# kije/gpu_raytracer

Measured on AMD Instinct MI355X. Metric: Mrays/s, higher is better.
Workload: dtype f32

## Files before the change

gpu_raytracer_amd/csrc/rt_frame.cpp:

```cpp
#include "rt_internal.h"

#ifndef RT_SINGLE_PASS_MAX_NODES
#define RT_SINGLE_PASS_MAX_NODES 64u
#endif
#ifndef RT_WF_LANES_DEFAULT
#define RT_WF_LANES_DEFAULT 2
#endif

namespace rti {
DevCamera make_camera(const rt_camera& cam, float res_x, float res_y, bool wavefront) {
    DevCamera c;
    float wf, hf;
    if (wavefront) {
        wf = res_x;
        hf = res_y;
    } else {
        auto as_u32 = [](float f) -> uint32_t { return !(f > 0.0f) ? 0u : (f >= 4294967296.0f ? 0xFFFFFFFFu : (uint32_t)f); };
        wf = (float)as_u32(res_x);
        hf = (float)as_u32(res_y);
    }
    c.width_f = wf;
    c.height_f = hf;
    c.aspect = wf / hf;
    c.fov_scale = tanf(cam.fov * 0.5f * 3.14159265358979323846f / 180.0f);
// ... 137 lines not shown
    const uint32_t ovf_entries = ctx->scene_counts.stack_entries + 2u > RT_WF8_LDS_STACK ? ctx->scene_counts.stack_entries + 2u - RT_WF8_LDS_STACK : 1u;
    const bool same_shape = shrink ? d.pipe.wf.n_blocks >= n_blocks : (d.pipe.wf.n_blocks == n_blocks && d.pipe.wf.batch == batch);
    if (d.pipe.wf.capacity >= capacity && same_shape && d.pipe.lights >= n_lights && d.pipe.wf.counters &&
        d.pipe.wf.ovf_entries >= ovf_entries && d.pipe.wf.stack_ovf && (!two_lanes || (d.pipe.wf2.counters && d.pipe.wf2.capacity >= capacity && d.pipe.wf2.stack_ovf)))
        return RT_OK;
    HIPCHK(ctx, hipSetDevice(d.device));
    d.pipe = {};
    DeviceState::Lanes fresh;
    for (int lane = 0; lane < (two_lanes ? 2 : 1); lane++) {
    std::vector<DevMem>& owned = lane ? fresh.allocs2 : fresh.allocs;
    auto alloc = [&](void** p, size_t bytes) -> hipError_t {
        owned.emplace_back();
        const hipError_t e = owned.back().reserve(bytes ? bytes : 16);
        *p = owned.back().get();
        return e;
    };
    rt::WfBuffers& w = lane ? fresh.wf2 : fresh.wf;
    const size_t P = capacity ? capacity : 64;
    const uint32_t lights = std::max(1u, n_lights);
    const size_t ext_slots = rt::wf_queue_slots(P, 1), shadow_slots = rt::wf_queue_slots(P * (size_t)lights, lights);
    if (ext_slots > 0xFFFFFFFFull || shadow_slots > 0xFFFFFFFFull)
        return ctx->fail(RT_ERR_INTERNAL, "wavefront queues of %zu / %zu slots exceed 32-bit positions", ext_slots, shadow_slots);
    const size_t S = std::min(rt::wf_state_slots(P), ext_slots);
    if (S > (size_t)RT_WF_ID_MASK + 1)
        return ctx->fail(RT_ERR_INTERNAL, "wavefront path ids of %zu slots exceed %u bits", S, 27u);
    HIPCHK(ctx, alloc((void**)&w.ray_o, S * 16));
    HIPCHK(ctx, alloc((void**)&w.ray_d, S * 16));
    HIPCHK(ctx, alloc((void**)&w.thr, S * 16));
    HIPCHK(ctx, alloc((void**)&w.rad, S * 16));
    HIPCHK(ctx, alloc((void**)&w.next_o, S * 16));
    HIPCHK(ctx, alloc((void**)&w.next_d, S * 16));
    HIPCHK(ctx, alloc((void**)&w.next_thr, S * 16));
    HIPCHK(ctx, alloc((void**)&w.next_rad, S * 16));
    HIPCHK(ctx, alloc((void**)&w.hit, S * 16));
    HIPCHK(ctx, alloc((void**)&w.vtx, S * 32));
    HIPCHK(ctx, alloc((void**)&w.sample_rad, P * 16));
    HIPCHK(ctx, alloc((void**)&w.pxy, P * 4));
    w.state_cap = (uint32_t)S;
    HIPCHK(ctx, alloc((void**)&w.q_ext[0], ext_slots * 4));
    HIPCHK(ctx, alloc((void**)&w.q_ext[1], ext_slots * 4));
    HIPCHK(ctx, alloc((void**)&w.q_shadow, shadow_slots * 4));
    HIPCHK(ctx, alloc((void**)&w.q_shadow2, (P * (size_t)lights + 64) * 4));
    w.q_ext_cap = (uint32_t)ext_slots;
    w.q_shadow_cap = (uint32_t)shadow_slots;
    HIPCHK(ctx, alloc((void**)&w.counters, rt::WF_N_COUNTERS * sizeof(uint32_t)));
    HIPCHK(ctx, alloc((void**)&w.totals, rt::WF_N_TOTALS * sizeof(unsigned long long)));
    if (lane == 0) HIPCHK(ctx, alloc((void**)&w.accum, (size_t)std::max(1u, n_blocks) * 64 * 16));
    else w.accum = fresh.wf.accum;
    if (lane == 0) {
        HIPCHK(ctx, alloc((void**)&w.beam_count, ((size_t)std::max(1u, n_blocks) + 1) * 4));
        HIPCHK(ctx, alloc((void**)&w.beam_ref, (size_t)std::max(1u, n_blocks) * RT_BEAM_CAP * 4));
        HIPCHK(ctx, alloc((void**)&w.beam_dist, (size_t)std::max(1u, n_blocks) * RT_BEAM_CAP * 4));
    } else {
        w.beam_count = fresh.wf.beam_count;
        w.beam_ref = fresh.wf.beam_ref;
        w.beam_dist = fresh.wf.beam_dist;
    }
    HIPCHK(ctx, alloc((void**)&w.stack_ovf, (size_t)rt::wf_persistent_waves() * ovf_entries * 64 * 8));
    w.ovf_entries = ovf_entries;
    w.n_blocks = n_blocks;
    w.batch = batch;
    w.capacity = capacity;
    }
    fresh.lights = n_lights;
    d.pipe = std::move(fresh);
    return RT_OK;
}

uint64_t wavefront_max_paths(uint32_t n_lights) {
    static const uint64_t by_ids = [] {
        uint64_t lo = 1, hi = (uint64_t)RT_WF_ID_MASK + 1;
        while (lo < hi) {
            const uint64_t mid = (lo + hi + 1) / 2;
            if (rt::wf_state_slots((size_t)mid) <= (uint64_t)RT_WF_ID_MASK + 1) lo = mid;
            else hi = mid - 1;
        }
        return lo;
    }();
    const uint64_t lights = std::max(1u, n_lights);
    return std::min<uint64_t>(by_ids, (1ull << 29) / lights);
}

uint32_t wavefront_batch(uint32_t n_blocks, uint32_t spp, uint32_t n_lights, size_t free_bytes, bool two_lanes) {
    const uint64_t per_sample = std::max<uint64_t>(1, (uint64_t)n_blocks * 64u);
    const uint64_t hard_limit = std::max<uint64_t>(1, wavefront_max_paths(n_lights) / per_sample);
    if (const char* e = std::getenv("RT_WF_BATCH")) {
        const uint32_t want = (uint32_t)std::strtoul(e, nullptr, 10);
        if (want) return (uint32_t)std::max<uint64_t>(1, std::min<uint64_t>(std::min(want, spp), hard_limit));
    }
    uint64_t target_paths = 64ull << 20;
    if (const char* e = std::getenv("RT_WF_TARGET_PATHS")) target_paths = std::max<uint64_t>(1, std::strtoull(e, nullptr, 10));
    const uint64_t lights = std::max(1u, n_lights);
    const uint64_t bytes_per_path = 2 * 11 * 16 + 16 + 4 + 2 * 16 + 16 * lights + 4 * lights;
    target_paths = std::min<uint64_t>(target_paths, free_bytes / 2 / bytes_per_path);
    target_paths = std::min<uint64_t>(target_paths, wavefront_max_paths(n_lights));
    uint32_t max_batch = (uint32_t)std::max<uint64_t>(1, std::min<uint64_t>(spp, target_paths / per_sample));
    if (two_lanes && spp >= 2) max_batch = std::min(max_batch, (spp + 1) / 2);
    uint32_t n_batches = (spp + max_batch - 1) / max_batch;
    if (two_lanes && n_batches > 1 && (n_batches & 1u)) {
        const uint32_t fewer = n_batches - 1, b = (spp + fewer - 1) / fewer;
        if ((uint64_t)b * per_sample * 10 <= target_paths * 11 && b <= hard_limit && (uint64_t)b * per_sample <= free_bytes / 2 / bytes_per_path) n_batches = fewer;
        else n_batches++;
    }
    return std::max(1u, (spp + n_batches - 1) / std::max(1u, n_batches));
}

uint32_t single_pass_max_nodes() {
    if (const char* e = std::getenv("RT_SINGLE_PASS_MAX_NODES")) return (uint32_t)std::strtoul(e, nullptr, 10);
    return RT_SINGLE_PASS_MAX_NODES;
}

void assign_tiles(DevFrame& f, DeviceState& d, uint32_t world, uint32_t rank, size_t nd, size_t j) {
    frame_share(f, world, rank, nd, j);
    d.tile_first = f.tile_first;
    d.tile_stride = f.tile_stride;
    d.n_owned = f.n_owned_tiles;
}

struct KernelChoice {
    rt::FrameKernel kernel;
    bool fallback;
};

KernelChoice choose_kernel(const rt_ctx* ctx, const DevFrame& f) {
    using rt::FrameKernel;
    const DevScene& sc = ctx->scene_counts;
// ... 429 lines not shown
```

gpu_raytracer_amd/csrc/wavefront.h:

```cpp
#ifndef RT_WAVEFRONT_H
#define RT_WAVEFRONT_H

#include <hip/hip_runtime.h>

#include "../../include/rt_hip.h"
#include "device_layout.h"
#include "shadow_grid.h"

namespace rt {

enum WfCounter : uint32_t {
    WF_EXT_COUNT = 0,
    WF_EXT_NEXT = 1,
    WF_SHADOW2_COUNT = 2,
    WF_SHADOW_COUNT = 3,
    WF_EXT_CURSOR = 4,
    WF_SHADOW_CURSOR = 5,
    WF_EXT_WINDOW = 6,
    WF_SHADOW_WINDOW = 7,
    WF_EXT_WINDOW_NEXT = 8,
    WF_SHADOW2_CURSOR = 9,
    WF_SHADOW2_WINDOW = 10,
    WF_UNUSED_11 = 11,
    WF_FB_COUNT = 12,
    WF_FB_CURSOR = 13,
    WF_N_COUNTERS = 16
};

enum WfTotal : uint32_t {
    WF_TOTAL_CAMERA = 0,
    WF_TOTAL_CONTINUATION = 1,
    WF_TOTAL_SHADOW = 2,
    WF_TOTAL_NODE_VISITS = 3,
    WF_TOTAL_TRI_TESTS = 4,
    WF_TOTAL_STACK_MAX = 5,
    WF_TOTAL_EMPTY_VISITS = 6,
    WF_TOTAL_CHILDREN_ENTERED = 7,
    WF_TOTAL_NODE_STEPS = 8,
    WF_TOTAL_LEAF_STEPS = 9,
    WF_TOTAL_LEAF_LANES = 10,
    WF_TOTAL_LEAF_TRIPS = 11,
    WF_TOTAL_REFILLS = 12,
    WF_TOTAL_GRID_ANSWERED = 13,
    WF_TOTAL_GRID_ENTRIES = 14,
    WF_TOTAL_ERROR = 15,
    WF_N_TOTALS = 16
};

struct WfBuffers {
    float4* ray_o;
    float4* ray_d;
    uint4* hit;
    float4* thr;
    float4* rad;
    float4* next_o;
    float4* next_d;
    float4* next_thr;
    float4* next_rad;
    float4* vtx;
    float4* sample_rad;
    uint32_t* pxy;
    uint32_t* q_ext[2];
    uint32_t* q_shadow;
    uint32_t* q_shadow2;
    const DevShadowGrid* grids;
    uint32_t* counters;
    unsigned long long* totals;
    float4* accum;
    uint32_t q_ext_cap;
    uint32_t q_shadow_cap;
    uint32_t state_cap;
    uint32_t* stack_ovf;
    uint32_t ovf_entries;
    uint32_t n_blocks;
    uint32_t batch;
    uint32_t capacity;
    uint32_t* beam_count;
    uint32_t* beam_ref;
    float* beam_dist;
    uint32_t probe;
};

#ifndef RT_BEAM_CAP
#define RT_BEAM_CAP 128u
#endif
// ... 25 lines not shown
```

gpu_raytracer_amd/csrc/wavefront.hip:

```cpp
#include "wavefront.h"
#include <cstdlib>

#include <algorithm>

#include "device_common.h"
#include "shadow_grid_walk.h"

using namespace rtdev;

#ifndef RT_WF_REFILL
#define RT_WF_REFILL 16
#endif
#ifndef RT_WF_CHUNK
#define RT_WF_CHUNK 256
#endif
#ifndef RT_WF_ADAPTIVE_CHUNK
#define RT_WF_ADAPTIVE_CHUNK 1
#endif
#ifndef RT_WF_WINDOW
#define RT_WF_WINDOW 512
#endif
#ifndef RT_WF_BLOCK_MAJOR
#define RT_WF_BLOCK_MAJOR 1
#endif
#ifndef RT_WF_SHADE_WAVES
#define RT_WF_SHADE_WAVES 4
#endif
#ifndef RT_WF_WAVES_PER_CU
#define RT_WF_WAVES_PER_CU 24
#endif
#ifndef RT_WF_WAVES_SMALL
#define RT_WF_WAVES_SMALL 12u
#endif
#ifndef RT_WF_SHADOW_LIGHT_MAJOR
#define RT_WF_SHADOW_LIGHT_MAJOR 1
#endif

namespace {

__device__ __forceinline__ V3 f4v(float4 a) { return v3(a.x, a.y, a.z); }
#define RT_KEEP4_EARLY(v) asm volatile("" : "+v"((v).x), "+v"((v).y), "+v"((v).z), "+v"((v).w))

#ifndef RT_WF_WINDOW_MAX
#define RT_WF_WINDOW_MAX 16384u
#endif
__host__ __device__ inline uint32_t wf_min_window(uint32_t per_lane) {
    uint32_t w = RT_WF_WINDOW;
    while (w < 128u * per_lane) w <<= 1;
    return w;
}
__host__ __device__ inline uint32_t pick_window(uint32_t iters, uint32_t per_lane) {
    const uint32_t most = iters * WAVE * per_lane;
    uint32_t w = wf_min_window(per_lane);
    while (w < most / 4u && w < RT_WF_WINDOW_MAX) w <<= 1;
    return w;
}
struct OutWindow {
    uint32_t next, end;
};
#define WF_SENTINEL 0xFFFFFFFFu
__device__ __forceinline__ void window_close(uint32_t* __restrict__ queue, OutWindow& w) {
    for (uint32_t i = w.next + (threadIdx.x & 63u); i < w.end; i += WAVE) queue[i] = WF_SENTINEL;
    w.next = w.end;
}
#define WF_NO_SLOT 0xFFFFFFFFu
__device__ __forceinline__ uint32_t window_reserve(uint32_t* __restrict__ queue, uint32_t* __restrict__ counter, OutWindow& w, uint32_t window,
                                                  uint32_t mine, uint32_t incl, uint32_t total, uint32_t capacity, unsigned long long* __restrict__ error) {
    if (w.next + total > w.end) {
// ... 58 lines not shown
            wb.pxy[p] = px.x | (px.y << 16);
        } else {
            wb.pxy[p] = 0xFFFFFFFFu;
            wb.sample_rad[p] = make_float4(0.0f, 0.0f, 0.0f, 0.0f);
        }
        const uint32_t mine = px.valid ? 1u : 0u;
        const uint32_t incl = wave_incl_scan(mine), total = __shfl(incl, WAVE - 1, WAVE);
        if (total) {
            const uint32_t at = window_reserve(wb.q_ext[0], &wb.counters[rt::WF_EXT_COUNT], win, window, mine, incl, total, wb.q_ext_cap, &wb.totals[rt::WF_TOTAL_ERROR]);
            if (mine && at != WF_NO_SLOT) wb.q_ext[0][at] = p;
            real += mine;
        }
        if (wb.beam_count) {
            const uint32_t bc = wb.beam_count[b];
            if (bc & RT_BEAM_OVERFLOW) wb.q_ext[1][((size_t)(bc & ~RT_BEAM_OVERFLOW) * n_samples + k) * WAVE + lane] = px.valid ? p : WF_SENTINEL;
        }
    }
    window_close(wb.q_ext[0], win);
    const unsigned long long r = wave_sum(real);
    if (lane == 0 && r) atomicAdd(&wb.totals[rt::WF_TOTAL_CAMERA], r);
}

#ifndef RT_WF8_LDS_STACK
#define RT_WF8_LDS_STACK 8
#endif
#ifndef RT_WF8_MIN_WAVES
#define RT_WF8_MIN_WAVES 6
#endif
#ifndef RT_WF8_LEAF_THRESHOLD
#define RT_WF8_LEAF_THRESHOLD 24
#endif
#define WF8_KIND_T 0x80000000u
#define WF8_NONE 0xFFFFFFFFu

template <bool COUNT, bool ANY>
__global__ __launch_bounds__(WAVE, RT_WF8_MIN_WAVES) void k_wf_trace(DevScene sc, rt::WfBuffers wb, const uint32_t* __restrict__ queue, uint32_t count_slot,
                                                    uint32_t cursor_slot, uint32_t window_slot) {
    extern __shared__ uint32_t s_mem8[];
    if (wb.totals[rt::WF_TOTAL_ERROR] != 0ull) return;
    const uint32_t lane = threadIdx.x;
    uint2* __restrict__ stack = reinterpret_cast<uint2*>(s_mem8) + lane;
    uint8_t* __restrict__ lut = reinterpret_cast<uint8_t*>(s_mem8 + RT_WF8_LDS_STACK * 2 * WAVE);
    for (uint32_t e = lane; e < 2048u; e += WAVE) {
        const uint32_t oct = e >> 8, m = e & 255u;
        uint32_t best = 0u, best_key = 99u;
        for (uint32_t i = 0; i < 8u; i++)
            if (((m >> i) & 1u) && (i ^ oct) < best_key) best_key = i ^ oct, best = i;
        lut[e] = (uint8_t)best;
    }
    __syncthreads();
    uint2* __restrict__ ovf = reinterpret_cast<uint2*>(wb.stack_ovf) + (size_t)blockIdx.x * wb.ovf_entries * WAVE + lane;
    const uint4* __restrict__ nodes = reinterpret_cast<const uint4*>(sc.nodes);
    const uint32_t count = wb.counters[count_slot];
    const uint32_t window_mask = max(wb.counters[window_slot], 1u) - 1u;
    uint32_t* cursor = &wb.counters[cursor_slot];
#if RT_WF_ADAPTIVE_CHUNK
    uint32_t chunk = RT_WF_CHUNK;
    while (chunk > WAVE && (unsigned long long)chunk * gridDim.x > count) chunk >>= 1;
#else
    const uint32_t chunk = RT_WF_CHUNK;
#endif
    Counts cnt = {0u, 0u};
    int sp_max = 0;
    uint32_t d_node_steps = 0, d_leaf_steps = 0, d_leaf_lanes = 0, d_leaf_trips = 0, d_refills = 0;
    uint32_t d_empty = 0, d_entered = 0;
    bool second = false;

    bool active = false, exhausted = false;
    uint32_t chunk_next = 0, chunk_end = 0;
    uint32_t id = 0, li = 0;
    V3 o = v3(0.0f, 0.0f, 0.0f), d = o;
    FilterRay fray;
    fray.o = o;
    fray.inv = o;
    Hit hit;
    hit.t = RT_F32_MAX;
    hit.prim = RT_PRIM_MISS;
    hit.slot = 0;
    uint32_t cur = WF8_NONE;
    uint32_t g_base = 0, g_bits = 0;
    uint32_t t_base = 0, t_bits = 0;
    uint32_t oct = 0;
    int sp = 0;

    for (;;) {
        const unsigned long long idle = __ballot(!active);
        if (!exhausted && (__popcll(idle) >= RT_WF_REFILL || idle == ~0ull)) {
            if (chunk_next >= chunk_end) {
                uint32_t base = 0;
                if (lane == 0) base = atomicAdd(cursor, chunk);
                base = __shfl(base, 0, WAVE);
                chunk_next = base;
                chunk_end = min(base + chunk, count);
                if (base >= count) exhausted = true;
            }
            if (!exhausted) {
                if (COUNT) d_refills++;
                const uint32_t n_fetch = (uint32_t)__popcll(idle);
                const uint32_t idx = chunk_next + (uint32_t)__popcll(idle & ((1ull << lane) - 1ull));
                const uint32_t last = min(chunk_next + n_fetch, chunk_end) - 1u;
                chunk_next += n_fetch;
                uint32_t e = WF_SENTINEL;
                if (!active && idx < chunk_end) e = queue[idx];
                if (__ballot(!active && idx == last && e == WF_SENTINEL) != 0ull) chunk_next = max(chunk_next, (last + window_mask + 1u) & ~window_mask);
                if (e != WF_SENTINEL) {
                    if (ANY) {
                        id = e & RT_WF_ID_MASK;
                        li = e >> 27;
                        const V3 point = f4v(wb.vtx[2 * (size_t)id]), normal = f4v(wb.vtx[2 * (size_t)id + 1]);
                        float dist;
                        shadow_segment(sc.lights[li], point, d, dist);
                        o = point + normal * EXT_EPS;
                        hit.t = dist;
                    } else {
                        id = e;
                        o = f4v(wb.ray_o[id]);
                        d = f4v(wb.ray_d[id]);
                        hit.t = RT_F32_MAX;
                    }
                    hit.prim = RT_PRIM_MISS;
                    hit.slot = 0;
                    fray = make_filter_ray(o, d);
                    oct = ((fray.inv.x < 0.0f ? 1u : 0u) | (fray.inv.y < 0.0f ? 2u : 0u) | (fray.inv.z < 0.0f ? 4u : 0u)) << 8;
                    if (ANY) oct ^= 7u << 8;
                    test_spheres(sc, o, d, hit, RT_MIN_RAY_DISTANCE);
                    sp = 0;
                    cur = WF8_NONE;
                    t_bits = 0;
                    g_base = 0;
                    g_bits = sc.n_nodes ? (1u | (1u << 8)) : 0u;
                    active = true;
                    if (ANY && hit.prim != RT_PRIM_MISS) g_bits = t_bits = 0;
                }
            }
        }
        if (__ballot(active) == 0ull) {
// ... 64 lines not shown
                    const uint32_t before = cnt.tris;
                    const uint32_t i = lut[oct + (t_bits & 0xFFu)];
                    t_bits ^= 1u << i;
                    const uint32_t first = t_base + RT_DEV_LEAF_STRIDE * (uint32_t)__popc(__builtin_amdgcn_ubfe(t_bits, 8u, i));
                    if (test_leaf<COUNT, ANY>(sc.tris, RT_DEV_LEAF_FLAG | first, o, d, hit, cnt, RT_MIN_RAY_DISTANCE)) {
                        cur = WF8_NONE;
                        g_bits = t_bits = 0u;
                        sp = 0;
                    }
                    trips = cnt.tris - before;
                    if (COUNT && wb.probe && !ANY && !second) cnt.tris = before;
                }
                if (COUNT) {
                    d_leaf_steps++;
                    d_leaf_lanes += (uint32_t)__popcll(m_leaf);
                    for (int off = 32; off > 0; off >>= 1) trips = max(trips, (uint32_t)__shfl_xor((int)trips, off, WAVE));
                    d_leaf_trips += trips;
                }
            }
            uint32_t busy = ((g_bits | t_bits) & 0xFFu) | (uint32_t)sp | (cur + 1u);
            if (COUNT && !ANY && wb.probe && active && busy == 0u && !second) {
                second = true;
                hit.t = fminf(hit.t * 1.00001f, RT_F32_MAX);
                hit.prim = RT_PRIM_MISS;
                g_base = 0;
                g_bits = sc.n_nodes ? (1u | (1u << 8)) : 0u;
                busy = g_bits & 0xFFu;
            }
            if (active && busy == 0u) {
                second = false;
                if (ANY) {
                    if (hit.prim != RT_PRIM_MISS) atomicAnd(reinterpret_cast<uint32_t*>(&wb.vtx[2 * (size_t)id + 1]) + 3, ~(1u << li));
                } else {
                    const V3 hp = o + d * hit.t;
                    const uint32_t code = hit.prim == RT_PRIM_MISS ? RT_PRIM_MISS : ((hit.prim & RT_PRIM_SPHERE_FLAG) ? hit.prim : hit.slot);
                    wb.hit[id] = make_uint4(__float_as_uint(hp.x), __float_as_uint(hp.y), __float_as_uint(hp.z), code);
                }
                active = false;
            }
            const unsigned long long still = __builtin_amdgcn_uicmp(busy, 0u, 33 );
            if (still == 0ull) break;
            if (!exhausted && __popcll(~still) >= RT_WF_REFILL) break;
        }
    }
    if (COUNT) {
        unsigned long long n0 = wave_sum(cnt.nodes), n1 = wave_sum(cnt.tris);
        for (int off = 32; off > 0; off >>= 1) sp_max = max(sp_max, __shfl_down(sp_max, off, WAVE));
        if (lane == 0) {
            atomicAdd(&wb.totals[rt::WF_TOTAL_NODE_VISITS], n0);
            atomicAdd(&wb.totals[rt::WF_TOTAL_TRI_TESTS], n1);
            atomicMax(&wb.totals[rt::WF_TOTAL_STACK_MAX], (unsigned long long)sp_max);
            atomicAdd(&wb.totals[rt::WF_TOTAL_NODE_STEPS], (unsigned long long)d_node_steps);
            atomicAdd(&wb.totals[rt::WF_TOTAL_LEAF_STEPS], (unsigned long long)d_leaf_steps);
            atomicAdd(&wb.totals[rt::WF_TOTAL_LEAF_LANES], (unsigned long long)d_leaf_lanes);
            atomicAdd(&wb.totals[rt::WF_TOTAL_LEAF_TRIPS], (unsigned long long)d_leaf_trips);
            atomicAdd(&wb.totals[rt::WF_TOTAL_REFILLS], (unsigned long long)d_refills);
        }
        const unsigned long long e0 = wave_sum(d_empty), e1 = wave_sum(d_entered);
        if (lane == 0) {
            atomicAdd(&wb.totals[rt::WF_TOTAL_EMPTY_VISITS], e0);
            atomicAdd(&wb.totals[rt::WF_TOTAL_CHILDREN_ENTERED], e1);
        }
    }
}

#ifndef RT_BEAM_STACK
#define RT_BEAM_STACK 512
#endif
#ifndef RT_BEAM_LEAVES
#define RT_BEAM_LEAVES 1024
#endif
#ifndef RT_BEAM_MARGIN_PX
#define RT_BEAM_MARGIN_PX 0.125f
#endif
#ifndef RT_BEAM_SAMPLES_PER_WAVE
#define RT_BEAM_SAMPLES_PER_WAVE 8u
#endif
// ... 173 lines not shown
        const uint32_t b = item / chunks, k_first = (item - b * chunks) * RT_BEAM_SAMPLES_PER_WAVE, k_end = min(n_samples, k_first + RT_BEAM_SAMPLES_PER_WAVE);
        const uint32_t n_list = (uint32_t)__builtin_amdgcn_readfirstlane((int)wb.beam_count[b]);
        if (n_list & RT_BEAM_OVERFLOW) continue;
        {
            __syncthreads();
            for (uint32_t i = lane; i < n_list; i += WAVE) {
                const uint32_t slot = wb.beam_ref[(size_t)b * RT_BEAM_CAP + i];
                const uint4* __restrict__ rec = reinterpret_cast<const uint4*>(sc.tris + slot);
                const uint4 q0 = rec[0], q1 = rec[1], q2 = rec[2];
                s_cam[3u * i] = q0;
                s_cam[3u * i + 1u] = q1;
                s_cam[3u * i + 2u] = make_uint4(q2.x, q2.y, q2.z, slot);
                s_d[i] = wb.beam_dist[(size_t)b * RT_BEAM_CAP + i];
            }
            __syncthreads();
        }
        for (uint32_t k = k_first; k < k_end; k++) {
            const uint32_t sb = RT_WF_BLOCK_MAJOR ? b * n_samples + k : k * wb.n_blocks + b;
            const uint32_t p = sb * WAVE + lane;
            const bool valid = wb.pxy[p] != 0xFFFFFFFFu;
            if (__ballot(valid) == 0ull) continue;
            V3 o = v3(0.0f, 0.0f, 0.0f), d = v3(0.0f, 0.0f, 1.0f);
            if (valid) {
                float4 ro = wb.ray_o[p], rd = wb.ray_d[p];
                RT_KEEP4_EARLY(ro);
                RT_KEEP4_EARLY(rd);
                o = f4v(ro);
                d = f4v(rd);
            }
            Hit hit;
            hit.t = valid ? RT_F32_MAX : -1.0f;
            hit.prim = RT_PRIM_MISS;
            hit.slot = 0;
            if (valid) test_spheres(sc, o, d, hit, RT_MIN_RAY_DISTANCE);
            {
                for (uint32_t i = 0; i < n_list; i++) {
                    if (RT_BEAM_EARLY_OUT && __ballot(s_d[i] < hit.t) == 0ull) break;
                    const uint4 q0 = s_cam[3u * i], q1 = s_cam[3u * i + 1u], q2 = s_cam[3u * i + 2u];
                    if (COUNT && valid) cnt.tris++;
                    float t = 0.0f;
                    const bool inside = moller_trumbore(v3(__uint_as_float(q0.x), __uint_as_float(q0.y), __uint_as_float(q0.z)), v3(__uint_as_float(q0.w), __uint_as_float(q1.x), __uint_as_float(q1.y)),
                                                        v3(__uint_as_float(q1.z), __uint_as_float(q1.w), __uint_as_float(q2.x)), o, d, t);
                    const uint32_t prim = q2.z;
                    const bool accept = inside && t > RT_MIN_RAY_DISTANCE && (t < hit.t || (t == hit.t && prim < hit.prim && hit.prim < RT_PRIM_SPHERE_FLAG));
                    hit.t = accept ? t : hit.t;
                    hit.prim = accept ? prim : hit.prim;
                    hit.slot = accept ? q2.w : hit.slot;
                }
            }
            if (COUNT && wb.probe == 2u && valid) {
                Hit h2;
                h2.t = RT_F32_MAX;
                h2.prim = RT_PRIM_MISS;
                h2.slot = 0;
                Counts c2 = {0u, 0u};
                test_spheres(sc, o, d, h2, RT_MIN_RAY_DISTANCE);
                traverse<false, false>(sc, o, d, reinterpret_cast<uint2*>(s_cam + RT_BEAM_CAP * 4u) + lane, h2, c2, RT_MIN_RAY_DISTANCE);
                if (h2.prim != hit.prim || h2.t != hit.t) {
                    if (atomicAdd(&wb.totals[rt::WF_TOTAL_EMPTY_VISITS], 1ull) == 0ull) {
                        wb.totals[rt::WF_TOTAL_NODE_STEPS] = b;
                        wb.totals[rt::WF_TOTAL_LEAF_STEPS] = ((unsigned long long)hit.prim << 32) | h2.prim;
                        wb.totals[rt::WF_TOTAL_LEAF_LANES] = ((unsigned long long)__float_as_uint(hit.t) << 32) | __float_as_uint(h2.t);
                        wb.totals[rt::WF_TOTAL_LEAF_TRIPS] = ((unsigned long long)n_list << 32) | h2.slot;
                        wb.totals[rt::WF_TOTAL_REFILLS] = p;
                    }
                }
            }
            if (valid) {
                const V3 hp = o + d * hit.t;
                const uint32_t code = hit.prim == RT_PRIM_MISS ? RT_PRIM_MISS : ((hit.prim & RT_PRIM_SPHERE_FLAG) ? hit.prim : hit.slot);
                wb.hit[p] = make_uint4(__float_as_uint(hp.x), __float_as_uint(hp.y), __float_as_uint(hp.z), code);
            }
        }
    }
    if (COUNT) {
        const unsigned long long n0 = wave_sum(cnt.nodes), n1 = wave_sum(cnt.tris);
        if (lane == 0) {
            atomicAdd(&wb.totals[rt::WF_TOTAL_NODE_VISITS], n0);
            atomicAdd(&wb.totals[rt::WF_TOTAL_TRI_TESTS], n1);
        }
    }
}

__device__ __forceinline__ DevMaterial load_material(const DevScene& sc, uint32_t material_id) {
    const float4* p = reinterpret_cast<const float4*>(sc.materials + material_id);
    float4 a = p[0], b = p[1];
    RT_KEEP4(a);
    RT_KEEP4(b);
    DevMaterial m;
    m.albedo[0] = a.x; m.albedo[1] = a.y; m.albedo[2] = a.z; m.metallic = a.w;
    m.emission[0] = b.x; m.emission[1] = b.y; m.emission[2] = b.z; m.ior = b.w;
    const float2 c = *reinterpret_cast<const float2*>(reinterpret_cast<const float*>(sc.materials + material_id) + 8);
    m.transmission = c.x; m.roughness = c.y;
    m._pad[0] = m._pad[1] = 0.0f;
    return m;
}

#ifndef RT_WF_GRID_BLOCKS_PER_CU
#define RT_WF_GRID_BLOCKS_PER_CU 32
#endif
#ifndef RT_WF_GRID_MIN_WAVES
#define RT_WF_GRID_MIN_WAVES 7
#endif

#ifndef RT_WF_GRID_PASS
#define RT_WF_GRID_PASS 3u
#endif
#define RT_WF_GRID_PARK 128u
#define RT_WF_GRID_PARK_WORDS 11u
template <bool COUNT>
__global__ __launch_bounds__(256, RT_WF_GRID_MIN_WAVES) void k_wf_shadow_grid(DevScene sc, rt::WfBuffers wb, const uint32_t* __restrict__ queue) {
    __shared__ DevLight s_lights[RT_WF_MAX_LIGHTS];
    __shared__ DevShadowGrid s_grids[RT_WF_MAX_LIGHTS];
    __shared__ uint32_t s_fwd[4][128];
    __shared__ uint32_t s_park[4][RT_WF_GRID_PARK_WORDS][RT_WF_GRID_PARK];
    if (wb.totals[rt::WF_TOTAL_ERROR] != 0ull) return;
    const uint32_t lane = threadIdx.x & 63u, wave = threadIdx.x >> 6;
    const unsigned long long below = (1ull << lane) - 1ull;
    uint32_t n_fwd = 0, n_park = 0;
    stage_lights(s_lights, sc);
    {
        const uint32_t words = sc.n_lights * (uint32_t)(sizeof(DevShadowGrid) / 4);
        const uint32_t* __restrict__ src = reinterpret_cast<const uint32_t*>(wb.grids);
        uint32_t* dst = reinterpret_cast<uint32_t*>(s_grids);
        for (uint32_t i = threadIdx.x; i < words; i += blockDim.x) dst[i] = src[i];
        __syncthreads();
    }
    uint32_t n_tests = 0, n_entries = 0, n_answered = 0;
    uint32_t(*park)[RT_WF_GRID_PARK] = s_park[wave];
    auto hand_on = [&](bool forward, uint32_t entry, bool flush) {
        const unsigned long long fm = __ballot(forward);
        if (fm != 0ull) {
            if (forward) s_fwd[wave][n_fwd + (uint32_t)__popcll(fm & below)] = entry;
            n_fwd += (uint32_t)__popcll(fm);
        }
        if (n_fwd >= 64u || (flush && n_fwd)) {
            uint32_t at = 0;
            if (lane == 0) at = atomicAdd(&wb.counters[rt::WF_SHADOW2_COUNT], n_fwd);
            at = __shfl(at, 0, WAVE);
            for (uint32_t k = lane; k < n_fwd; k += WAVE) wb.q_shadow2[at + k] = s_fwd[wave][k];
            n_fwd = 0;
        }
    };
    auto park_push = [&](bool pending, const GridPending& pd, uint32_t entry) {
        const unsigned long long pm = __ballot(pending);
        if (pm == 0ull) return;
        if (pending) {
            const uint32_t s = n_park + (uint32_t)__popcll(pm & below);
            park[0][s] = __float_as_uint(pd.o.x), park[1][s] = __float_as_uint(pd.o.y), park[2][s] = __float_as_uint(pd.o.z);
            park[3][s] = __float_as_uint(pd.d.x), park[4][s] = __float_as_uint(pd.d.y), park[5][s] = __float_as_uint(pd.d.z);
            park[6][s] = __float_as_uint(pd.dist), park[7][s] = __float_as_uint(pd.limit);
            park[8][s] = pd.at, park[9][s] = pd.i | (pd.count << 8), park[10][s] = entry;
        }
        n_park += (uint32_t)__popcll(pm);
    };
    auto walk_parked = [&]() {
        const uint32_t take = min(n_park, 64u), first = n_park - take;
        const bool have = lane < take;
        GridPending pd = {};
        uint32_t entry = 0, outcome = GRID_VISIBLE;
        if (have) {
            const uint32_t s = first + lane;
            pd.o = v3(__uint_as_float(park[0][s]), __uint_as_float(park[1][s]), __uint_as_float(park[2][s]));
            pd.d = v3(__uint_as_float(park[3][s]), __uint_as_float(park[4][s]), __uint_as_float(park[5][s]));
            pd.dist = __uint_as_float(park[6][s]), pd.limit = __uint_as_float(park[7][s]);
            pd.at = park[8][s];
            const uint32_t ic = park[9][s];
            pd.i = ic & 0xFFu, pd.count = ic >> 8;
            entry = park[10][s];
            outcome = grid_walk_on<COUNT>(s_grids[entry >> 27], pd, RT_WF_GRID_PASS, n_tests, n_entries);
            if (outcome == GRID_OCCLUDED) atomicAnd(reinterpret_cast<uint32_t*>(&wb.vtx[2 * (size_t)(entry & RT_WF_ID_MASK) + 1]) + 3, ~(1u << (entry >> 27)));
            if (COUNT && outcome <= GRID_OCCLUDED) n_answered++;
        }
        n_park = first;
        park_push(have && outcome == GRID_PENDING, pd, entry);
        hand_on(have && outcome == GRID_FORWARD, entry, false);
    };
    const uint32_t count = wb.counters[rt::WF_EXT_COUNT];
    const uint32_t stride = gridDim.x * blockDim.x;
    uint32_t id_next = blockIdx.x * blockDim.x + threadIdx.x < count ? queue[blockIdx.x * blockDim.x + threadIdx.x] : WF_SENTINEL;
    for (uint32_t base = blockIdx.x * blockDim.x; base < count; base += stride) {
        const uint32_t id = id_next;
        const uint32_t i_next = base + stride + threadIdx.x;
        id_next = i_next < count ? queue[i_next] : WF_SENTINEL;
        uint32_t want = 0;
        V3 point = v3(0, 0, 0), normal = point;
        if (id != WF_SENTINEL) {
            float4 vp = wb.vtx[2 * (size_t)id], vn = wb.vtx[2 * (size_t)id + 1];
            RT_KEEP4(vp);
            RT_KEEP4(vn);
            point = f4v(vp), normal = f4v(vn);
            if (__float_as_uint(vp.w) != 0xFFFFFFFFu) want = __float_as_uint(vn.w);
        }
        uint32_t occluded = 0;
        for (uint32_t li = 0; li < sc.n_lights; li++) {
            const bool mine = (want >> li) & 1u;
            if (__ballot(mine) == 0ull) continue;
            uint32_t outcome = GRID_VISIBLE;
            GridPending pd = {};
            if (mine) {
                outcome = grid_segment_head<COUNT>(sc, s_lights[li], s_grids[li], point, normal, pd, n_tests, n_entries);
                if (outcome == GRID_OCCLUDED) occluded |= 1u << li;
                if (COUNT && outcome <= GRID_OCCLUDED) n_answered++;
            }
            const uint32_t entry = id | (li << 27);
            park_push(mine && outcome == GRID_PENDING, pd, entry);
            hand_on(mine && outcome == GRID_FORWARD, entry, false);
            while (n_park >= 64u) walk_parked();
        }
        if (occluded != 0u) atomicAnd(reinterpret_cast<uint32_t*>(&wb.vtx[2 * (size_t)id + 1]) + 3, ~occluded);
    }
    while (n_park != 0u) walk_parked();
    hand_on(false, 0u, true);
    if (COUNT) {
        const unsigned long long t = wave_sum(n_tests), a = wave_sum(n_answered), en = wave_sum(n_entries);
        if ((threadIdx.x & 63u) == 0) {
            atomicAdd(&wb.totals[rt::WF_TOTAL_TRI_TESTS], t);
            atomicAdd(&wb.totals[rt::WF_TOTAL_GRID_ANSWERED], a);
            atomicAdd(&wb.totals[rt::WF_TOTAL_GRID_ENTRIES], en);
        }
    }
}

__device__ __forceinline__ void wf_end_path(const rt::WfBuffers& wb, uint32_t origin, V3 radiance) {
    wb.sample_rad[origin] = make_float4(radiance.x, radiance.y, radiance.z, 0.0f);
}
__device__ __forceinline__ uint32_t wf_origin(const rt::WfBuffers& wb, uint32_t id) { return __float_as_uint(wb.ray_d[id].w); }

__global__ __launch_bounds__(256, RT_WF_SHADE_WAVES) void k_wf_shade(DevScene sc, DevFrame fr, rt::WfBuffers wb, const uint32_t* __restrict__ queue) {
    __shared__ DevLight s_lights[RT_WF_MAX_LIGHTS];
    if (wb.totals[rt::WF_TOTAL_ERROR] != 0ull) return;
    stage_lights(s_lights, sc);
    const uint32_t count = wb.counters[rt::WF_EXT_COUNT];
    const bool shadows = (fr.flags & RT_FLAG_NO_SHADOWS) == 0;
    const bool to_grids = shadows && wb.grids != nullptr;
    const uint32_t stride = gridDim.x * blockDim.x;
    OutWindow win = {0u, 0u};
    uint32_t n_shadow = 0;
    const uint32_t window = pick_window((count + stride - 1u) / stride, max(1u, sc.n_lights));
    if (blockIdx.x == 0 && threadIdx.x == 0) wb.counters[rt::WF_SHADOW_WINDOW] = window;
    uint32_t id_next = blockIdx.x * blockDim.x + threadIdx.x < count ? queue[blockIdx.x * blockDim.x + threadIdx.x] : WF_SENTINEL;
    for (uint32_t base = blockIdx.x * blockDim.x; base < count; base += stride) {
        const uint32_t id = id_next;
        const uint32_t i_next = base + stride + threadIdx.x;
        id_next = i_next < count ? queue[i_next] : WF_SENTINEL;
        const bool have = id != WF_SENTINEL;
        bool vertex = false;
        V3 point = v3(0, 0, 0), normal = point;
        uint32_t material_id = 0;
        DevMaterial m = {};
        if (have) {
            uint4 h = wb.hit[id];
            asm volatile("" : "+v"(h.x), "+v"(h.y), "+v"(h.z), "+v"(h.w));
            if (h.w == RT_PRIM_MISS) {
                const V3 radiance = f4v(wb.rad[id]) + RT_SKY() * f4v(wb.thr[id]);
                wf_end_path(wb, wf_origin(wb, id), radiance);
            } else {
                point = v3(__uint_as_float(h.x), __uint_as_float(h.y), __uint_as_float(h.z));
                surface_at(sc, (h.w & RT_PRIM_SPHERE_FLAG) != 0, h.w & ~RT_PRIM_SPHERE_FLAG, point, normal, material_id);
                if (material_id >= sc.n_materials) {
                    const V3 radiance = f4v(wb.rad[id]) + RT_MAGENTA() * f4v(wb.thr[id]);
                    wf_end_path(wb, wf_origin(wb, id), radiance);
                } else {
                    vertex = true;
                    m = load_material(sc, material_id);
                    wb.vtx[2 * (size_t)id] = make_float4(point.x, point.y, point.z, __uint_as_float(material_id));
                    if (!shadows) wb.vtx[2 * (size_t)id + 1] = make_float4(normal.x, normal.y, normal.z, 0.0f);
                }
            }
        }
        if (have && !vertex) wb.vtx[2 * (size_t)id] = make_float4(0.0f, 0.0f, 0.0f, __uint_as_float(0xFFFFFFFFu));
        if (shadows) {
            uint32_t mask = 0;
            if (vertex) {
                for (uint32_t li = 0; li < sc.n_lights; li++) {
                    V3 sdir;
                    float sdist;
                    const V3 contrib = light_contribution(s_lights[li], m, point, normal, sdir, sdist);
                    if (needs_shadow_segment(contrib)) mask |= 1u << li;
                }
            }
            if (vertex) wb.vtx[2 * (size_t)id + 1] = make_float4(normal.x, normal.y, normal.z, __uint_as_float(mask));
            if (to_grids) {
                n_shadow += (uint32_t)__popc(mask);
                continue;
            }
#if RT_WF_SHADOW_LIGHT_MAJOR
            uint32_t total = 0;
            for (uint32_t li = 0; li < sc.n_lights; li++) total += (uint32_t)__popcll(__ballot((mask >> li) & 1u));
            if (total) {
                uint32_t at = window_reserve(wb.q_shadow, &wb.counters[rt::WF_SHADOW_COUNT], win, window, 0u, 0u, total, wb.q_shadow_cap, &wb.totals[rt::WF_TOTAL_ERROR]);
                n_shadow += (uint32_t)__popc(mask);
                const unsigned long long below = (1ull << (threadIdx.x & 63u)) - 1ull;
                for (uint32_t li = 0; at != WF_NO_SLOT && li < sc.n_lights; li++) {
                    const bool want = (mask >> li) & 1u;
                    const unsigned long long b = __ballot(want);
                    if (want) wb.q_shadow[at + (uint32_t)__popcll(b & below)] = id | (li << 27);
                    at += (uint32_t)__popcll(b);
                }
            }
#else
            const uint32_t mine = (uint32_t)__popc(mask);
            const uint32_t incl = wave_incl_scan(mine), total = __shfl(incl, WAVE - 1, WAVE);
            if (total) {
                uint32_t at = window_reserve(wb.q_shadow, &wb.counters[rt::WF_SHADOW_COUNT], win, window, mine, incl, total, wb.q_shadow_cap, &wb.totals[rt::WF_TOTAL_ERROR]);
                n_shadow += mine;
                while (mask && at != WF_NO_SLOT) {
                    const uint32_t li = (uint32_t)__ffs((int)mask) - 1u;
                    mask &= mask - 1u;
                    wb.q_shadow[at++] = id | (li << 27);
                }
            }
#endif
        }
    }
// ... 20 lines not shown
    __shared__ DevLight s_lights[RT_WF_MAX_LIGHTS];
    if (wb.totals[rt::WF_TOTAL_ERROR] != 0ull) return;
    stage_lights(s_lights, sc);
    const uint32_t count = wb.counters[rt::WF_EXT_COUNT];
    const bool shadows = (fr.flags & RT_FLAG_NO_SHADOWS) == 0;
    const uint32_t stride = gridDim.x * blockDim.x;
    OutWindow win = {0u, 0u};
    uint32_t n_cont = 0;
    const uint32_t window = pick_window((count + stride - 1u) / stride, 1u);
    if (blockIdx.x == 0 && threadIdx.x == 0) wb.counters[rt::WF_EXT_WINDOW_NEXT] = window;
    uint32_t id_next = blockIdx.x * blockDim.x + threadIdx.x < count ? queue[blockIdx.x * blockDim.x + threadIdx.x] : WF_SENTINEL;
    for (uint32_t base = blockIdx.x * blockDim.x; base < count; base += stride) {
        bool cont = false;
        V3 norigin = v3(0.0f, 0.0f, 0.0f), ndir = norigin, throughput = norigin, radiance = norigin;
        uint32_t next_tw = 0, rng_seed = 0, ndir_origin = 0;
        const uint32_t id = id_next;
        const uint32_t i_next = base + stride + threadIdx.x;
        id_next = i_next < count ? queue[i_next] : WF_SENTINEL;
        float4 vp = make_float4(0.0f, 0.0f, 0.0f, __uint_as_float(0xFFFFFFFFu));
        float4 vn = vp, th = vp, ra = vp, rdin = vp;
        if (id != WF_SENTINEL) {
            vp = wb.vtx[2 * (size_t)id];
            vn = wb.vtx[2 * (size_t)id + 1];
            th = wb.thr[id];
            ra = wb.rad[id];
            rdin = wb.ray_d[id];
            RT_KEEP4(vp);
            RT_KEEP4(vn);
            RT_KEEP4(th);
            RT_KEEP4(ra);
            RT_KEEP4(rdin);
        }
        const uint32_t vis = __float_as_uint(vn.w);
        if (__float_as_uint(vp.w) != 0xFFFFFFFFu) {
            const V3 point = f4v(vp), normal = f4v(vn);
            const uint32_t material_id = __float_as_uint(vp.w);
            const uint32_t origin = __float_as_uint(rdin.w);
            const DevMaterial m = load_material(sc, material_id);
            throughput = f4v(th), radiance = f4v(ra);
            const uint32_t tw = __float_as_uint(th.w);
            uint32_t channel = tw & 0xFFu;
            const uint32_t depth = tw >> 8;
            SimpleRng rng = {__float_as_uint(ra.w)};
            const bool terminal = depth >= fr.max_bounce;
            const V3 lighting = ext_light_sum(s_lights, sc.n_lights, m, point, normal, terminal, shadows, [&](uint32_t li, V3, float) { return ((vis >> li) & 1u) != 0u; });
            const float tf = ext_leave_vertex(m, lighting, terminal, throughput, radiance);
            if (terminal || !ext_scatter(m, point, normal, f4v(rdin), tf, depth, rng, channel, throughput, norigin, ndir)) {
                wf_end_path(wb, origin, radiance);
            } else {
                cont = true;
                next_tw = channel | ((depth + 1u) << 8);
                rng_seed = rng.seed;
                ndir_origin = origin;
            }
        }
        const uint32_t mine = cont ? 1u : 0u;
        const uint32_t incl = wave_incl_scan(mine), total = __shfl(incl, WAVE - 1, WAVE);
        if (total) {
            const uint32_t at = window_reserve(next_queue, &wb.counters[rt::WF_EXT_NEXT], win, window, mine, incl, total, wb.state_cap, &wb.totals[rt::WF_TOTAL_ERROR]);
            if (cont && at != WF_NO_SLOT) {
                wb.next_o[at] = make_float4(norigin.x, norigin.y, norigin.z, 0.0f);
                wb.next_d[at] = make_float4(ndir.x, ndir.y, ndir.z, __uint_as_float(ndir_origin));
                wb.next_thr[at] = make_float4(throughput.x, throughput.y, throughput.z, __uint_as_float(next_tw));
                wb.next_rad[at] = make_float4(radiance.x, radiance.y, radiance.z, __uint_as_float(rng_seed));
                next_queue[at] = at;
            }
            n_cont += mine;
// ... 120 lines not shown
    else hipLaunchKernelGGL(k_wf_generate<false>, dim3(wf_shading_blocks()), dim3(256), 0, s, fr, wb, tg, first_sample, n_samples * wb.n_blocks);
    return hipGetLastError();
}

template <bool COUNT, bool ANY>
static void launch_trace(const DevScene& sc, const WfBuffers& wb, const uint32_t* q, uint32_t count_slot, uint32_t cursor_slot, uint32_t window_slot, hipStream_t s) {
    const size_t lds = (size_t)RT_WF8_LDS_STACK * WAVE * sizeof(uint2) + 2048;
    hipLaunchKernelGGL((k_wf_trace<COUNT, ANY>), dim3((uint32_t)cu_count() * trace_waves_per_cu(wb.capacity)), dim3(WAVE), lds, s, sc, wb, q, count_slot, cursor_slot, window_slot);
}

hipError_t wf_bounce(const DevScene& sc, const DevFrame& fr, const WfBuffers& wb_in, uint32_t iteration, uint32_t n_samples, bool counters, hipStream_t s, hipEvent_t* grid_events) {
    const dim3 sgrid(wf_shading_blocks()), sblock(256);
    WfBuffers wb = wb_in;
    if (iteration & 1u) {
        std::swap(wb.ray_o, wb.next_o);
        std::swap(wb.ray_d, wb.next_d);
        std::swap(wb.thr, wb.next_thr);
        std::swap(wb.rad, wb.next_rad);
    }
    uint32_t* cur_q = wb.q_ext[iteration & 1u];
    uint32_t* next_q = wb.q_ext[(iteration + 1u) & 1u];
    if (iteration == 0 && wb.beam_count && n_samples && wb.n_blocks) {
        const dim3 lgrid(std::min<uint32_t>(wb.n_blocks * ((n_samples + RT_BEAM_SAMPLES_PER_WAVE - 1u) / RT_BEAM_SAMPLES_PER_WAVE), (uint32_t)cu_count() * 96u));
        const size_t list_lds = (size_t)RT_BEAM_CAP * (3 * sizeof(uint4) + sizeof(float)), walk_lds = (size_t)std::max(1u, sc.stack_entries) * WAVE * sizeof(uint2);
        if (counters) {
            hipLaunchKernelGGL((k_wf_trace_camera<true>), lgrid, dim3(WAVE), wb.probe == 2u ? (size_t)RT_BEAM_CAP * 64 + walk_lds : list_lds, s, sc, wb, n_samples);
            launch_trace<true, false>(sc, wb, wb.q_ext[1], WF_FB_COUNT, WF_FB_CURSOR, WF_SHADOW2_WINDOW, s);
        } else {
            hipLaunchKernelGGL((k_wf_trace_camera<false>), lgrid, dim3(WAVE), list_lds, s, sc, wb, n_samples);
            launch_trace<false, false>(sc, wb, wb.q_ext[1], WF_FB_COUNT, WF_FB_CURSOR, WF_SHADOW2_WINDOW, s);
        }
    } else if (counters) launch_trace<true, false>(sc, wb, cur_q, WF_EXT_COUNT, WF_EXT_CURSOR, WF_EXT_WINDOW, s);
    else launch_trace<false, false>(sc, wb, cur_q, WF_EXT_COUNT, WF_EXT_CURSOR, WF_EXT_WINDOW, s);
    hipLaunchKernelGGL(k_wf_shade, sgrid, sblock, 0, s, sc, fr, wb, (const uint32_t*)cur_q);
    if (wf_runs_shadow_grid(fr, wb)) {
        const dim3 ggrid((uint32_t)(cu_count() * RT_WF_GRID_BLOCKS_PER_CU));
        if (grid_events) (void)hipEventRecord(grid_events[0], s);
        if (counters) hipLaunchKernelGGL(k_wf_shadow_grid<true>, ggrid, dim3(256), 0, s, sc, wb, (const uint32_t*)cur_q);
        else hipLaunchKernelGGL(k_wf_shadow_grid<false>, ggrid, dim3(256), 0, s, sc, wb, (const uint32_t*)cur_q);
        if (grid_events) (void)hipEventRecord(grid_events[1], s);
        if (counters) launch_trace<true, true>(sc, wb, wb.q_shadow2, WF_SHADOW2_COUNT, WF_SHADOW2_CURSOR, WF_SHADOW2_WINDOW, s);
        else launch_trace<false, true>(sc, wb, wb.q_shadow2, WF_SHADOW2_COUNT, WF_SHADOW2_CURSOR, WF_SHADOW2_WINDOW, s);
    } else if ((fr.flags & RT_FLAG_NO_SHADOWS) == 0) {
        if (counters) launch_trace<true, true>(sc, wb, wb.q_shadow, WF_SHADOW_COUNT, WF_SHADOW_CURSOR, WF_SHADOW_WINDOW, s);
        else launch_trace<false, true>(sc, wb, wb.q_shadow, WF_SHADOW_COUNT, WF_SHADOW_CURSOR, WF_SHADOW_WINDOW, s);
    }
    hipLaunchKernelGGL(k_wf_finish, sgrid, sblock, 0, s, sc, fr, wb, (const uint32_t*)cur_q, next_q);
    hipLaunchKernelGGL(k_wf_advance, dim3(1), dim3(1), 0, s, wb);
    return hipGetLastError();
}

hipError_t wf_resolve(const DevFrame& fr, const WfBuffers& wb, const DevTargets& tg, uint32_t n_samples, uint32_t first_sample, bool first_batch, bool last_batch,
                      hipStream_t s) {
    if (wb.n_blocks == 0) return hipSuccess;
    if (fr.adaptive)
        hipLaunchKernelGGL(k_wf_resolve<true>, dim3(wb.n_blocks), dim3(WAVE), 0, s, fr, wb, tg, n_samples, first_sample, first_batch ? 1u : 0u, last_batch ? 1u : 0u);
    else
        hipLaunchKernelGGL(k_wf_resolve<false>, dim3(wb.n_blocks), dim3(WAVE), 0, s, fr, wb, tg, n_samples, first_sample, first_batch ? 1u : 0u, last_batch ? 1u : 0u);
    return hipGetLastError();
}

}
```

Before: 3282.

## Store shading vertex directly from trace kernels and skip shade pass with grid

The extension trace and camera trace kernels now compute the surface point, normal and material themselves and write the vertex record directly, which removes the intermediate hit buffer. Sky and magenta path terminations are encoded in the vertex record and resolved later in the finish kernel. The shade kernel is reduced to building shadow masks, and when the shadow grid runs it is skipped entirely because the grid kernel computes the light mask itself. This cuts one kernel launch and a round trip through global memory per bounce, at the cost of more work and register pressure inside the trace kernels, which could lower their occupancy.

```diff
diff --git a/gpu_raytracer_amd/csrc/rt_frame.cpp b/gpu_raytracer_amd/csrc/rt_frame.cpp
--- a/gpu_raytracer_amd/csrc/rt_frame.cpp
+++ b/gpu_raytracer_amd/csrc/rt_frame.cpp
@@ -193,7 +193,6 @@
     HIPCHK(ctx, alloc((void**)&w.next_d, S * 16));
     HIPCHK(ctx, alloc((void**)&w.next_thr, S * 16));
     HIPCHK(ctx, alloc((void**)&w.next_rad, S * 16));
-    HIPCHK(ctx, alloc((void**)&w.hit, S * 16));
     HIPCHK(ctx, alloc((void**)&w.vtx, S * 32));
     HIPCHK(ctx, alloc((void**)&w.sample_rad, P * 16));
     HIPCHK(ctx, alloc((void**)&w.pxy, P * 4));
@@ -252,7 +251,7 @@
     uint64_t target_paths = 64ull << 20;
     if (const char* e = std::getenv("RT_WF_TARGET_PATHS")) target_paths = std::max<uint64_t>(1, std::strtoull(e, nullptr, 10));
     const uint64_t lights = std::max(1u, n_lights);
-    const uint64_t bytes_per_path = 2 * 11 * 16 + 16 + 4 + 2 * 16 + 16 * lights + 4 * lights;
+    const uint64_t bytes_per_path = 2 * 10 * 16 + 16 + 4 + 2 * 16 + 16 * lights + 4 * lights;
     target_paths = std::min<uint64_t>(target_paths, free_bytes / 2 / bytes_per_path);
     target_paths = std::min<uint64_t>(target_paths, wavefront_max_paths(n_lights));
     uint32_t max_batch = (uint32_t)std::max<uint64_t>(1, std::min<uint64_t>(spp, target_paths / per_sample));
diff --git a/gpu_raytracer_amd/csrc/wavefront.h b/gpu_raytracer_amd/csrc/wavefront.h
--- a/gpu_raytracer_amd/csrc/wavefront.h
+++ b/gpu_raytracer_amd/csrc/wavefront.h
@@ -50,7 +50,6 @@
 struct WfBuffers {
     float4* ray_o;
     float4* ray_d;
-    uint4* hit;
     float4* thr;
     float4* rad;
     float4* next_o;
diff --git a/gpu_raytracer_amd/csrc/wavefront.hip b/gpu_raytracer_amd/csrc/wavefront.hip
--- a/gpu_raytracer_amd/csrc/wavefront.hip
+++ b/gpu_raytracer_amd/csrc/wavefront.hip
@@ -34,6 +34,9 @@
 #endif
 #ifndef RT_WF_SHADOW_LIGHT_MAJOR
 #define RT_WF_SHADOW_LIGHT_MAJOR 1
+#endif
+#ifndef RT_WF_GRID_MASK
+#define RT_WF_GRID_MASK 1
 #endif
 
 namespace {
@@ -158,6 +161,20 @@
 #endif
 #define WF8_KIND_T 0x80000000u
 #define WF8_NONE 0xFFFFFFFFu
+
+#define WF_NO_VERTEX 0xFFFFFFFFu
+#define WF_END_SKY 0u
+#define WF_END_MAGENTA 1u
+__device__ __forceinline__ uint32_t wf_all_lights(uint32_t n_lights) { return n_lights >= RT_WF_MAX_LIGHTS ? 0xFFFFFFFFu : (1u << n_lights) - 1u; }
+__device__ __forceinline__ void wf_store_vertex(const DevScene& sc, const rt::WfBuffers& wb, uint32_t id, bool found, V3 point, V3 normal, uint32_t material_id) {
+    float4* __restrict__ rec = wb.vtx + 2 * (size_t)id;
+    if (found && material_id < sc.n_materials) {
+        rec[0] = make_float4(point.x, point.y, point.z, __uint_as_float(material_id));
+        rec[1] = make_float4(normal.x, normal.y, normal.z, __uint_as_float(wf_all_lights(sc.n_lights)));
+    } else {
+        rec[0] = make_float4(__uint_as_float(found ? WF_END_MAGENTA : WF_END_SKY), 0.0f, 0.0f, __uint_as_float(WF_NO_VERTEX));
+    }
+}
 
 template <bool COUNT, bool ANY>
 __global__ __launch_bounds__(WAVE, RT_WF8_MIN_WAVES) void k_wf_trace(DevScene sc, rt::WfBuffers wb, const uint32_t* __restrict__ queue, uint32_t count_slot,
@@ -208,6 +225,20 @@
     uint32_t t_base = 0, t_bits = 0;
     uint32_t oct = 0;
     int sp = 0;
+    bool pending = false;
+    auto write_pending = [&]() {
+        if (ANY || !pending) return;
+        const bool found = hit.prim != RT_PRIM_MISS;
+        V3 hp = v3(0.0f, 0.0f, 0.0f), normal = hp;
+        uint32_t material_id = 0;
+        if (found) {
+            hp = o + d * hit.t;
+            const uint32_t code = (hit.prim & RT_PRIM_SPHERE_FLAG) ? hit.prim : hit.slot;
+            surface_at(sc, (code & RT_PRIM_SPHERE_FLAG) != 0, code & ~RT_PRIM_SPHERE_FLAG, hp, normal, material_id);
+        }
+        wf_store_vertex(sc, wb, id, found, hp, normal, material_id);
+        pending = false;
+    };
 
     for (;;) {
         const unsigned long long idle = __ballot(!active);
@@ -228,6 +259,7 @@
                 chunk_next += n_fetch;
                 uint32_t e = WF_SENTINEL;
                 if (!active && idx < chunk_end) e = queue[idx];
+                write_pending();
                 if (__ballot(!active && idx == last && e == WF_SENTINEL) != 0ull) chunk_next = max(chunk_next, (last + window_mask + 1u) & ~window_mask);
                 if (e != WF_SENTINEL) {
                     if (ANY) {
@@ -358,9 +390,7 @@
                 if (ANY) {
                     if (hit.prim != RT_PRIM_MISS) atomicAnd(reinterpret_cast<uint32_t*>(&wb.vtx[2 * (size_t)id + 1]) + 3, ~(1u << li));
                 } else {
-                    const V3 hp = o + d * hit.t;
-                    const uint32_t code = hit.prim == RT_PRIM_MISS ? RT_PRIM_MISS : ((hit.prim & RT_PRIM_SPHERE_FLAG) ? hit.prim : hit.slot);
-                    wb.hit[id] = make_uint4(__float_as_uint(hp.x), __float_as_uint(hp.y), __float_as_uint(hp.z), code);
+                    pending = true;
                 }
                 active = false;
             }
@@ -369,6 +399,7 @@
             if (!exhausted && __popcll(~still) >= RT_WF_REFILL) break;
         }
     }
+    write_pending();
     if (COUNT) {
         unsigned long long n0 = wave_sum(cnt.nodes), n1 = wave_sum(cnt.tris);
         for (int off = 32; off > 0; off >>= 1) sp_max = max(sp_max, __shfl_down(sp_max, off, WAVE));
@@ -608,6 +639,7 @@
             hit.t = valid ? RT_F32_MAX : -1.0f;
             hit.prim = RT_PRIM_MISS;
             hit.slot = 0;
+            uint32_t hit_i = 0;
             if (valid) test_spheres(sc, o, d, hit, RT_MIN_RAY_DISTANCE);
             {
                 for (uint32_t i = 0; i < n_list; i++) {
@@ -622,6 +654,7 @@
                     hit.t = accept ? t : hit.t;
                     hit.prim = accept ? prim : hit.prim;
                     hit.slot = accept ? q2.w : hit.slot;
+                    hit_i = accept ? i : hit_i;
                 }
             }
             if (COUNT && wb.probe == 2u && valid) {
@@ -643,9 +676,22 @@
                 }
             }
             if (valid) {
-                const V3 hp = o + d * hit.t;
-                const uint32_t code = hit.prim == RT_PRIM_MISS ? RT_PRIM_MISS : ((hit.prim & RT_PRIM_SPHERE_FLAG) ? hit.prim : hit.slot);
-                wb.hit[p] = make_uint4(__float_as_uint(hp.x), __float_as_uint(hp.y), __float_as_uint(hp.z), code);
+                const bool found = hit.prim != RT_PRIM_MISS;
+                V3 hp = v3(0.0f, 0.0f, 0.0f), normal = hp;
+                uint32_t material_id = 0;
+                if (found) {
+                    hp = o + d * hit.t;
+                    if (hit.prim & RT_PRIM_SPHERE_FLAG) {
+                        surface_at(sc, true, hit.prim & ~RT_PRIM_SPHERE_FLAG, hp, normal, material_id);
+                    } else {
+                        const uint4 q0 = s_cam[3u * hit_i], q1 = s_cam[3u * hit_i + 1u], q2 = s_cam[3u * hit_i + 2u];
+                        const V3 e1 = v3(__uint_as_float(q0.w), __uint_as_float(q1.x), __uint_as_float(q1.y));
+                        const V3 e2 = v3(__uint_as_float(q1.z), __uint_as_float(q1.w), __uint_as_float(q2.x));
+                        normal = normalize(cross(e1, e2));
+                        material_id = q2.y;
+                    }
+                }
+                wf_store_vertex(sc, wb, p, found, hp, normal, material_id);
             }
         }
     }
@@ -703,6 +749,9 @@
         __syncthreads();
     }
     uint32_t n_tests = 0, n_entries = 0, n_answered = 0;
+#if RT_WF_GRID_MASK
+    uint32_t n_want = 0;
+#endif
     uint32_t(*park)[RT_WF_GRID_PARK] = s_park[wave];
     auto hand_on = [&](bool forward, uint32_t entry, bool flush) {
         const unsigned long long fm = __ballot(forward);
@@ -766,7 +815,22 @@
             RT_KEEP4(vp);
             RT_KEEP4(vn);
             point = f4v(vp), normal = f4v(vn);
-            if (__float_as_uint(vp.w) != 0xFFFFFFFFu) want = __float_as_uint(vn.w);
+            if (__float_as_uint(vp.w) != WF_NO_VERTEX) {
+#if RT_WF_GRID_MASK
+                float4 a = *reinterpret_cast<const float4*>(sc.materials + __float_as_uint(vp.w));
+                RT_KEEP4(a);
+                DevMaterial m = {};
+                m.albedo[0] = a.x, m.albedo[1] = a.y, m.albedo[2] = a.z, m.metallic = a.w;
+                for (uint32_t li = 0; li < sc.n_lights; li++) {
+                    V3 sdir;
+                    float sdist;
+                    if (needs_shadow_segment(light_contribution(s_lights[li], m, point, normal, sdir, sdist))) want |= 1u << li;
+                }
+                n_want += (uint32_t)__popc(want);
+#else
+                want = __float_as_uint(vn.w);
+#endif
+            }
         }
         uint32_t occluded = 0;
         for (uint32_t li = 0; li < sc.n_lights; li++) {
@@ -788,6 +852,12 @@
     }
     while (n_park != 0u) walk_parked();
     hand_on(false, 0u, true);
+#if RT_WF_GRID_MASK
+    {
+        const unsigned long long ns = wave_sum(n_want);
+        if (lane == 0 && ns) atomicAdd(&wb.totals[rt::WF_TOTAL_SHADOW], ns);
+    }
+#endif
     if (COUNT) {
         const unsigned long long t = wave_sum(n_tests), a = wave_sum(n_answered), en = wave_sum(n_entries);
         if ((threadIdx.x & 63u) == 0) {
@@ -801,15 +871,13 @@
 __device__ __forceinline__ void wf_end_path(const rt::WfBuffers& wb, uint32_t origin, V3 radiance) {
     wb.sample_rad[origin] = make_float4(radiance.x, radiance.y, radiance.z, 0.0f);
 }
-__device__ __forceinline__ uint32_t wf_origin(const rt::WfBuffers& wb, uint32_t id) { return __float_as_uint(wb.ray_d[id].w); }
-
-__global__ __launch_bounds__(256, RT_WF_SHADE_WAVES) void k_wf_shade(DevScene sc, DevFrame fr, rt::WfBuffers wb, const uint32_t* __restrict__ queue) {
+
+__global__ __launch_bounds__(256, RT_WF_SHADE_WAVES) void k_wf_shade(DevScene sc, rt::WfBuffers wb, const uint32_t* __restrict__ queue) {
     __shared__ DevLight s_lights[RT_WF_MAX_LIGHTS];
     if (wb.totals[rt::WF_TOTAL_ERROR] != 0ull) return;
     stage_lights(s_lights, sc);
     const uint32_t count = wb.counters[rt::WF_EXT_COUNT];
-    const bool shadows = (fr.flags & RT_FLAG_NO_SHADOWS) == 0;
-    const bool to_grids = shadows && wb.grids != nullptr;
+    const bool to_grids = wb.grids != nullptr;
     const uint32_t stride = gridDim.x * blockDim.x;
     OutWindow win = {0u, 0u};
     uint32_t n_shadow = 0;
@@ -820,43 +888,26 @@
         const uint32_t id = id_next;
         const uint32_t i_next = base + stride + threadIdx.x;
         id_next = i_next < count ? queue[i_next] : WF_SENTINEL;
-        const bool have = id != WF_SENTINEL;
-        bool vertex = false;
-        V3 point = v3(0, 0, 0), normal = point;
-        uint32_t material_id = 0;
-        DevMaterial m = {};
-        if (have) {
-            uint4 h = wb.hit[id];
-            asm volatile("" : "+v"(h.x), "+v"(h.y), "+v"(h.z), "+v"(h.w));
-            if (h.w == RT_PRIM_MISS) {
-                const V3 radiance = f4v(wb.rad[id]) + RT_SKY() * f4v(wb.thr[id]);
-                wf_end_path(wb, wf_origin(wb, id), radiance);
-            } else {
-                point = v3(__uint_as_float(h.x), __uint_as_float(h.y), __uint_as_float(h.z));
-                surface_at(sc, (h.w & RT_PRIM_SPHERE_FLAG) != 0, h.w & ~RT_PRIM_SPHERE_FLAG, point, normal, material_id);
-                if (material_id >= sc.n_materials) {
-                    const V3 radiance = f4v(wb.rad[id]) + RT_MAGENTA() * f4v(wb.thr[id]);
-                    wf_end_path(wb, wf_origin(wb, id), radiance);
-                } else {
-                    vertex = true;
-                    m = load_material(sc, material_id);
-                    wb.vtx[2 * (size_t)id] = make_float4(point.x, point.y, point.z, __uint_as_float(material_id));
-                    if (!shadows) wb.vtx[2 * (size_t)id + 1] = make_float4(normal.x, normal.y, normal.z, 0.0f);
-                }
-            }
-        }
-        if (have && !vertex) wb.vtx[2 * (size_t)id] = make_float4(0.0f, 0.0f, 0.0f, __uint_as_float(0xFFFFFFFFu));
-        if (shadows) {
+        {
             uint32_t mask = 0;
-            if (vertex) {
-                for (uint32_t li = 0; li < sc.n_lights; li++) {
-                    V3 sdir;
-                    float sdist;
-                    const V3 contrib = light_contribution(s_lights[li], m, point, normal, sdir, sdist);
-                    if (needs_shadow_segment(contrib)) mask |= 1u << li;
-                }
-            }
-            if (vertex) wb.vtx[2 * (size_t)id + 1] = make_float4(normal.x, normal.y, normal.z, __uint_as_float(mask));
+            if (id != WF_SENTINEL) {
+                float4 vp = wb.vtx[2 * (size_t)id], vn = wb.vtx[2 * (size_t)id + 1];
+                RT_KEEP4(vp);
+                RT_KEEP4(vn);
+                if (__float_as_uint(vp.w) != WF_NO_VERTEX) {
+                    float4 a = *reinterpret_cast<const float4*>(sc.materials + __float_as_uint(vp.w));
+                    RT_KEEP4(a);
+                    DevMaterial m = {};
+                    m.albedo[0] = a.x, m.albedo[1] = a.y, m.albedo[2] = a.z, m.metallic = a.w;
+                    for (uint32_t li = 0; li < sc.n_lights; li++) {
+                        V3 sdir;
+                        float sdist;
+                        const V3 contrib = light_contribution(s_lights[li], m, f4v(vp), f4v(vn), sdir, sdist);
+                        if (needs_shadow_segment(contrib)) mask |= 1u << li;
+                    }
+                    reinterpret_cast<uint32_t*>(&wb.vtx[2 * (size_t)id + 1])[3] = mask;
+                }
+            }
             if (to_grids) {
                 n_shadow += (uint32_t)__popc(mask);
                 continue;
@@ -943,7 +994,10 @@
             RT_KEEP4(rdin);
         }
         const uint32_t vis = __float_as_uint(vn.w);
-        if (__float_as_uint(vp.w) != 0xFFFFFFFFu) {
+        if (id != WF_SENTINEL && __float_as_uint(vp.w) == WF_NO_VERTEX) {
+            const V3 end = __float_as_uint(vp.x) == WF_END_SKY ? RT_SKY() : RT_MAGENTA();
+            wf_end_path(wb, __float_as_uint(rdin.w), f4v(ra) + end * f4v(th));
+        } else if (__float_as_uint(vp.w) != WF_NO_VERTEX) {
             const V3 point = f4v(vp), normal = f4v(vn);
             const uint32_t material_id = __float_as_uint(vp.w);
             const uint32_t origin = __float_as_uint(rdin.w);
@@ -1130,7 +1184,7 @@
         }
     } else if (counters) launch_trace<true, false>(sc, wb, cur_q, WF_EXT_COUNT, WF_EXT_CURSOR, WF_EXT_WINDOW, s);
     else launch_trace<false, false>(sc, wb, cur_q, WF_EXT_COUNT, WF_EXT_CURSOR, WF_EXT_WINDOW, s);
-    hipLaunchKernelGGL(k_wf_shade, sgrid, sblock, 0, s, sc, fr, wb, (const uint32_t*)cur_q);
+    if ((fr.flags & RT_FLAG_NO_SHADOWS) == 0 && !(RT_WF_GRID_MASK && wf_runs_shadow_grid(fr, wb))) hipLaunchKernelGGL(k_wf_shade, sgrid, sblock, 0, s, sc, wb, (const uint32_t*)cur_q);
     if (wf_runs_shadow_grid(fr, wb)) {
         const dim3 ggrid((uint32_t)(cu_count() * RT_WF_GRID_BLOCKS_PER_CU));
         if (grid_events) (void)hipEventRecord(grid_events[0], s);
```

Result: faster. 3459 (median of 6 runs) (+5.4%).
